# karenyang/GCN-VAE

Measured on AMD Instinct MI355X. Metric: edges/sec R-GCN forward+backward, FB15k-237 emb=200, higher is better.
Workload: dtype f32; 1 GPU; FB15k-237-shaped synthetic full graph (BASELINE configs[1]): 14541 entities, 474 directed relation types, E=544230 directed edges on this rank (544230 in the trained graph), 2-layer R-GCN-VAE bdd num_bases=100 emb_dim=200 dropout 0.2, 0 IAF blocks, DistMult decoder on T=220000 triplets per rank, step = fwd + loss(BCE+reg+KL+MMD) + bwd + clip + Adam; edges_per_gpu=544230, trained_graph_edges=544230, nodes=14541, triplets_per_gpu=220000, n_flows=0, gemm_precision=f32, launch=hipgraph, parallelism=single GPU, optimizer=replicated clip + Adam, k1_operands=f32

## Files before the change

gcn-vae_amd/lib.py:

```python
import ctypes
import os

import torch

_HERE = os.path.dirname(os.path.abspath(__file__))
LIB_PATH = os.path.join(_HERE, 'libgcnvae_hip.so')

_P, _I, _L, _F = ctypes.c_void_p, ctypes.c_int, ctypes.c_int64, ctypes.c_float

SIGNATURES = {
    'gv_version': (_I, []),
    'gv_last_error_string': (ctypes.c_char_p, []),
    'gv_index_caps': (None, [_L, _I, _I, _P, _P, _P]),
    'gv_index_workspace_bytes': (_L, [_L, _I]),
    'gv_build_csr': (_I, [_P, _L, _I, _I, _P, _P, _P, _I, _P, _I, _P, _L, _P]),
    'gv_build_csr_batch_workspace_bytes': (_L, [_P, _I]),
    'gv_build_csr_batch': (_I, [_P, _I, _P, _L, _P]),
    'gv_triplet_lists': (_I, [_P, _I, _L, _P, _P, _P, _P, _P, _P, _P, _P, _P]),
    'gv_widen2_i32': (_I, [_P, _P, _L, _P, _P, _L, _P]),
    'gv_graph_index_build': (_I, [_P, _P, _L, _I, _I, _I, _I, _P, _P, _P, _P, _I, _P, _I, _P, _P, _P, _P, _I, _P, _I, _P, _L, _P]),
    'gv_relation_index_build': (_I, [_P, _P, _P, _P, _P, _L, _I, _I, _P, _P, _P, _P, _P, _P, _P, _I, _P, _I, _P, _L, _P]),
    'gv_triplet_index_build': (_I, [_P, _L, _I, _I, _I, _I, _P, _P, _P, _P, _P, _I, _P, _I, _P, _P, _P, _P, _P, _I, _P, _I,
                                    _P, _L, _P]),
    'gv_perm_sample': (_I, [_L, _L, ctypes.c_uint64, ctypes.c_uint64, _P, _P, ctypes.c_uint32, _P, _P]),
    'gv_neighborhood_sample_workspace_bytes': (_L, [_I, _L]),
    'gv_neighborhood_sample': (_I, [_P, _P, _P, _P, _I, _L, _I, ctypes.c_uint64, ctypes.c_uint64, _P, ctypes.c_uint32, _P, _P, _L, _P]),
    'gv_relabel_workspace_bytes': (_L, [_I]),
    'gv_relabel_pairs': (_I, [_P, _P, _L, _I, _P, _I, _P, _P, _P, _P, _L, _P]),
    'gv_negative_sampling': (_I, [_P, _P, _P, _L, _I, _P, _P, _P, ctypes.c_uint64, ctypes.c_uint64, _P, ctypes.c_uint32, _P, _P, _P]),
    'gv_graph_from_triplets_workspace_bytes': (_L, [_L, _I, _I]),
    'gv_graph_from_triplets': (_I, [_P, _P, _P, _P, _L, _I, _I, _P, _P, _P, _P, _P, _L, _P]),
    'gv_segment_items_count': (_I, [_P, _I, _I, _P, _P, _P, _P]),
    'gv_segment_items_fill': (_I, [_P, _I, _I, _P, _P, _P, _P, _P, _P]),
    'gv_rgcn_bdd_aggregate': (_I, [_P, _I, _P, _I, _P, _P, _P, _P, _P, _I, _P, _I, _I, _I, _I, _I, _I,
                                   _P, _I, _I, _P, _F, _P, _I, _P, _P]),
    'gv_rgcn_bdd_phase_plan': (_I, [_I, _I, _I, _I, _I, _I, _I, _I, _I, _P]),
    'gv_rgcn_bdd_pack_weight_phase': (_I, [_P, _I, _I, _I, _I, _I, _P, _P]),
    'gv_rgcn_bdd_aggregate_phases': (_I, [_P, _P, _P, _P, _P, _I, _P, _I, _P, _I, _P, _I, _I, _I, _I, _I, _I, _I, _I, _I,
                                          _P, _I, _I, _P, _F, _P, _I, _P, _P]),
    'gv_rgcn_bdd_lds_plan': (_I, [_I, _I, _I, _I, _I, _P]),
    'gv_rgcn_bdd_pack_weight_lds': (_I, [_P, _I, _I, _I, _I, _I, _I, _P, _P]),
    'gv_rgcn_bdd_aggregate_lds': (_I, [_P, _I, _P, _P, _I, _P, _I, _P, _P, _P, _P, _P, _I, _P, _I, _I, _I, _I, _I, _P, _I, _I,
                                       _P, _F, _P, _I, _P, _I, _P]),
    'gv_rgcn_bdd_pack_supported': (_I, [_I, _I, _I, _I]),
    'gv_rgcn_bdd_pack_weight': (_I, [_P, _I, _I, _I, _I, _I, _P, _P]),
    'gv_rgcn_bdd_pack_weight_pair': (_I, [_P, _I, _I, _I, _I, _P, _P, _P]),
    'gv_rgcn_bdd_fixup': (_I, [_P, _I, _P, _I, _P, _I, _I, _P, _F, _P, _I, _P]),
    'gv_rgcn_bdd_grad_weight': (_I, [_P, _I, _P, _I, _P, _P, _P, _P, _P, _I, _P, _I, _I, _I, _I, _P, _P, _I, _P]),
    'gv_rgcn_epilogue_fwd': (_I, [_P, _P, _I, _P, _F, _P, _L, _I, _P]),
    'gv_rgcn_epilogue_bwd': (_I, [_P, _P, _I, _P, _F, _P, _L, _I, _P, _P]),
    'gv_colsum_finish': (_I, [_P, _I, _I, _P, _I, _P]),
    'gv_gemm_workspace_bytes': (_L, [_I, _I, _I, _I]),
    'gv_gemm_f32': (_I, [_I, _I, _I, _I, _I, _P, _I, _P, _I, _P, _I, _P, _I, _I, _I, _P, _P, _L, _P]),
    'gv_gemm_f32_live_rows': (_I, [_I, _I, _I, _I, _I, _P, _I, _P, _I, _P, _I, _P, _I, _I, _I, _P, _P, _L, _P, _P]),
    'gv_gemm_f32_sparse': (_I, [_I, _I, _I, _I, _I, _P, _I, _P, _I, _P, _I, _P, _I, _I, _I, _P, _P, _L, _P, _P, _P, _I, _P]),
    'gv_gemm_bf16': (_I, [_I, _I, _I, _I, _I, _P, _I, _P, _I, _P, _I, _P, _I, _I, _I, _P, _P, _L, _P]),
    'gv_gemm_bf16_nt_workspace_bytes': (_L, [_I, _I, _I]),
    'gv_gemm_bf16_gradw_fits': (_I, [_I, _I, _I, _I]),
    'gv_gemm_bf16_gradw_workspace_bytes': (_L, [_I, _I, _I]),
    'gv_gemm_bf16_gradw': (_I, [_P, _I, _P, _I, _I, _I, _I, _P, _I, _P, _I, _P, _L, _P]),
    'gv_gemm_bf16_gradw_tiles': (_I, [_P, _L, _P, _L, _I, _I, _I, _P, _I, _P, _I, _P, _L, _P]),
    'gv_gemm_bf16_nt': (_I, [_P, _I, _I, _P, _I, _I, _I, _I, _P, _I, _P, _I, _P, _I, _I, _P, _I, _P, _I, _I, _P, _L, _P]),
    'gv_cast_bf16': (_I, [_P, _I, _I, _I, _P, _I, _P, _I, _P]),
    'gv_rowsum_bf16_workspace_floats': (_L, [_I, _I]),
    'gv_iaf_update_fwd_bf16': (_I, [_P, _P, _I, _P, _P, _P, _P, _I, _P, _I, _L, _I, _P]),
    'gv_iaf_update_fwd_bf16_tiles': (_I, [_P, _P, _I, _P, _P, _P, _P, _I, _P, _L, _L, _I, _P]),
    'gv_iaf_update_bwd_bf16': (_I, [_P, _P, _I, _P, _P, _P, _P, _P, _I, _P, _I, _P, _L, _I, _P]),
    'gv_gather3_i32': (_I, [_P, _L, _P, _P, _P, _P, _P, _P, _P]),
    'gv_iaf_update_bwd_row0_workspace_floats': (_L, [_I]),
    'gv_iaf_update_bwd_row0': (_I, [_P, _P, _P, _P, _P, _P, _P, _P, _L, _I, _P]),
    'gv_iaf_update_bwd_bf16_ex': (_I, [_P, _P, _I, _P, _P, _P, _P, _P, _I, _P, _I, _P, _I, _L, _I, _P]),
    'gv_rowsum_bf16': (_I, [_P, _I, _I, _I, _P, _I, _P, _P]),
    'gv_rowsum_bf16_segments': (_I, [_P, _I, _I, _I, _I, _P, _P, _I, _P, _P]),
    'gv_made_pack_weight_elems': (_L, [_I, _I]),
    'gv_made_pack_weight': (_I, [_P, _I, _I, _I, _P, _P, _P]),
    'gv_made_pack_weight_multi': (_I, [_I, _P, _P, _P, _P, _P, _P, _P]),
    'gv_made_pack_weight_multi_iaf': (_I, [_I, _P, _P, _P, _P, _P, _P, _P]),
    'gv_made_pack_weight_iaf': (_I, [_P, _I, _I, _I, _P, _P]),
    'gv_made_chain_fits': (_I, [_I, _P, _P, _I]),
    'gv_made_chain': (_I, [_P, _I, _I, _I, _P, _P]),
    'gv_made_chain_iafb': (_I, [_P, _I, _I, _P, _P]),
    'gv_made_chain_fwd': (_I, [_P, _I, _I, _I, _P, _I, _P, _P]),
    'gv_made_chain_fwd_row0': (_I, [_P, _I, _I, _P, _I, _P, _P]),
    'gv_made_chain_debug_stamps': (_I, [_P]),
    'gv_made_pack_weight_f32_elems': (_L, [_I, _I]),
    'gv_made_pack_weight_f32_multi': (_I, [_I, _P, _P, _P, _P, _P, _P, _P]),
    'gv_made_chain_f32_fits': (_I, [_I, _P, _P]),
    'gv_made_chain_f32_plan': (_I, [_I, _P, _P, _P, _P, _P, _P, _P]),
    'gv_made_chain_f32': (_I, [_P, _I, _I, _I, _P, _P, _P, _P]),
    'gv_made_passes_f32': (_I, [_P, _I, _I, _I, _P, _P, _P, _P, _P]),
    'gv_made_gradw_f32_plan_words': (_L, [_I, _I]),
    'gv_made_gradw_f32_plan': (_I, [_P, _I, _I, _I, _P, _P]),
    'gv_made_gradw_f32_workspace_floats': (_L, [_I, _I, _L]),
    'gv_made_gradw_f32': (_I, [_P, _I, _P, _I, _I, _I, _L, _P, _P, _I, _P, _P, _P, _P, _I, _I, _P, _I, _P, _L, _P]),
    'gv_made_gradw_f32_multi_workspace_floats': (_L, [_I, _P]),
    'gv_made_gradw_f32_multi': (_I, [_I, _P, _P, _L, _P]),
    'gv_made_row_fwd': (_I, [_P, _I, _P, _P]),
    'gv_made_row_bwd': (_I, [_P, _I, _P, _P, _P]),
    'gv_rel_rows_gemm': (_I, [_P, _I, _P, _P, _I, _I, _I, _I, _P, _I, _P, _P]),
    'gv_rel_gradw_gemm': (_I, [_P, _I, _P, _P, _I, _P, _P, _P, _I, _I, _I, _P, _P]),
    'gv_rank_scores': (_I, [_P, _I, _P, _I, _P, _P, _P, _P, _I, _I, _I, _P]),
    'gv_rank_scores_filtered': (_I, [_P, _I, _P, _I, _P, _P, _P, _P, _P, _I, _P, _P, _P, _I, _I, _I, _P]),
    'gv_topk_scores_workspace_bytes': (_L, [_I, _I, _I]),
    'gv_topk_scores': (_I, [_P, _I, _P, _I, _P, _P, _P, _P, _I, _I, _P, _P, _P, _I, _I, _I, _P]),
    'gv_rank_scores_constrained': (_I, [_P, _I, _P, _I, _P, _P, _P, _P, _P, _I, _P, _I, _I, _P, _P, _P, _P, _P, _P, _I, _I, _I, _P]),
    'gv_topk_scores_constrained': (_I, [_P, _I, _P, _I, _P, _P, _P, _P, _I, _P, _I, _I, _P, _I, _P, _P, _P, _I, _I, _I, _P]),
    'gv_rank_scores_mc': (_I, [_P, _I, _L, _P, _I, _L, _I, _P, _P, _P, _P, _P, _I, _P, _P, _P, _I, _I, _I, _P]),
    'gv_topk_scores_mc': (_I, [_P, _I, _L, _P, _I, _L, _I, _P, _P, _P, _P, _I, _I, _P, _P, _P, _I, _I, _I, _P]),
    'gv_pair_prob_std_mc': (_I, [_P, _I, _L, _P, _I, _L, _I, _P, _P, _I, _P, _I, _I, _I, _P]),
    'gv_mine_scores_workspace_bytes': (_L, [_I, _I, _I]),
    'gv_mine_scores': (_I, [_P, _I, _P, _I, _P, _P, _P, _P, _I, _I, _I, ctypes.c_uint32, _I, ctypes.c_uint32, _I, _P, _L, _P, _P, _P, _L,
                            _I, _I, _I, _P]),
    'gv_mine_scores_typed': (_I, [_P, _I, _P, _I, _P, _P, _P, _P, _L, _P, _P, _P, _I, _I, _I, ctypes.c_uint32, _I, ctypes.c_uint32, _I,
                                  _P, _L, _P, _P, _I, _I, _I, _P]),
    'gv_mine_scores_typed_mc': (_I, [_P, _I, _L, _I, _P, _I, _P, _P, _P, _P, _L, _P, _P, _P, _I, _I, _I, ctypes.c_uint32, _I,
                                     ctypes.c_uint32, _I, _P, _L, _P, _P, _I, _I, _I, _P]),
    'gv_ec_basis_rows_fwd': (_I, [_P, _P, _P, _P, _L, _I, _I, _I, _L, _P, _P]),
    'gv_ec_basis_rows_bwd': (_I, [_P, _P, _P, _P, _P, _P, _L, _P, _P, _L, _I, _I, _I, _L, _P, _P, _P, _I, _P]),
    'gv_ec_head_fwd': (_I, [_P, _P, _P, _P, _L, _I, _P, _P, _P, _P, _P, _P]),
    'gv_ec_head_bwd': (_I, [_P, _P, _P, _P, _P, _P, _L, _I, _P, _P]),
    'gv_transe_sample': (_I, [_P, ctypes.c_uint32, _P, _L, _I, _P, _P, _P, _P, _P, _I, _I, _P, _P, _P, _P, _P]),
    'gv_transe_step': (_I, [_P, _P, _P, _P, _P, _I, _I, _I, _I, _I, _F, _F, _F, _P, _P, _P, _P, _P, _P]),
    'gv_transe_apply': (_I, [_P, _I, _P, _P, _P, _P, _I, _P, _P, _P, _I, _F, _P, _I, _F, _P, _P, _P]),
    'gv_transe_apply_opt': (_I, [_P, _I, _P, _P, _P, _P, _I, _P, _P, _P, _I, _I, ctypes.c_double, ctypes.c_double, ctypes.c_double,
                                 _P, _P, _P, _P, _P, _P, _I, _F, _P, _P, _P]),
    'gv_transe_queries': (_I, [_P, _P, _P, _P, _L, _I, _I, _I, _P, _P]),
    'gv_transe_distances': (_I, [_P, _L, _P, _I, _I, _I, _P, _P]),
    'gv_transe_rank_filtered': (_I, [_P, _L, _P, _I, _I, _I, _P, _P, _P, _P, _P, _P, _P]),
    'gv_transe_topk_workspace_bytes': (_L, [_L, _I, _I]),
    'gv_transe_topk': (_I, [_P, _L, _P, _I, _I, _I, _P, _P, _P, _I, _I, _P, _P, _P, _P]),
    'gv_transe_rank_constrained': (_I, [_P, _L, _P, _I, _I, _I, _P, _P, _P, _P, _P, _I, _I, _P, _P, _P, _P, _P, _P]),
    'gv_transe_topk_constrained': (_I, [_P, _L, _P, _I, _I, _I, _P, _P, _P, _I, _P, _I, _I, _P, _I, _P, _P, _P, _P]),
    'gv_transe_mine_workspace_bytes': (_L, [_I, _I, _I]),
    'gv_transe_mine': (_I, [_P, _P, _I, _I, _I, _I, _P, _P, _P, _I, _I, _I, ctypes.c_uint32, _I, ctypes.c_uint32, _I, _P, _L, _P, _P,
                            _P, _L, _P]),
    'gv_transe_mine_typed': (_I, [_P, _P, _I, _I, _I, _I, _P, _P, _P, _L, _P, _P, _P, _I, _I, _I, ctypes.c_uint32, _I, ctypes.c_uint32,
                                  _I, _P, _L, _P, _P, _P]),
    'gv_colsum': (_I, [_P, _P, _L, _I, _I, _P, _P, _I, _P]),
    'gv_gather_rows': (_I, [_P, _P, _P, _L, _I, _P]),
# ... 102 lines not shown
```

gcn-vae_amd/ops.py:

```python
import contextlib
import ctypes as _ct
import itertools as _it
import os as _os
from dataclasses import dataclass
from typing import Optional

import torch

from . import lib
from .lib import ptr

ACT_NONE, ACT_RELU = 0, 1

DIRECT_GRAD = {}
GRAD_FRESH = set()
DIRECT_EPOCH = [0]


def _stamp_direct(ctx):
    ctx._gv_direct_epoch = DIRECT_EPOCH[0]


def _verify_direct(ctx):
    if getattr(ctx, '_gv_direct_epoch', DIRECT_EPOCH[0]) != DIRECT_EPOCH[0]:
# ... 891 lines not shown

MINE_TYPED_SPAN = 8
MINE_TYPED_FILL = 1024


def mine_typed_plan(ptr, num_rels, span=None, multiple=1):
    sizes = (ptr[1:] - ptr[:-1]).to(torch.int64)
    n_o, n_s = sizes[:num_rels], sizes[num_rels:]
    s_tiles, o_tiles = (n_s + 63) // 64, (n_o + 63) // 64
    if span is None:
        pairs = int((s_tiles * o_tiles).sum())
        span = min(MINE_TYPED_SPAN, max(1, pairs // MINE_TYPED_FILL))
        span = max(multiple, span // multiple * multiple)
    span = int(span)
    if span < 1:
        raise ValueError(f'span must be >= 1, got {span}')
    groups = (o_tiles + span - 1) // span
    per_r = s_tiles * groups
    total = int(per_r.sum())
    if total > 2 ** 31 - 1:
        raise ValueError(f'the type-constrained sweep has {total} units, more than 2**31 - 1')
    rel = torch.repeat_interleave(torch.arange(num_rels, device=ptr.device), per_r)
    local = torch.arange(total, device=ptr.device) - (torch.cumsum(per_r, 0) - per_r)[rel]
    g = groups[rel].clamp(min=1)
    first = (local % g) * span
    units = torch.stack([rel, local // g, first, torch.minimum(first + span, o_tiles[rel])], 1)
    return units.to(torch.int32).contiguous()


def _mine_typed_members(ptr, ids, n, num_rels):
    for name, t in (('ptr', ptr), ('ids', ids)):
        if not isinstance(t, torch.Tensor) or t.dim() != 1 or t.dtype not in (torch.int32, torch.int64):
            raise TypeError(f'{name}: expected a 1-D int32 / int64 tensor')
    if ptr.numel() != 2 * num_rels + 1:
        raise ValueError(f'ptr: expected {2 * num_rels + 1} entries (2 R + 1), got {ptr.numel()}')
    if ids.device != ptr.device:
        raise ValueError('ptr and ids must be on one device')
    ptr = ptr.to(torch.int64)
    if int(ptr[0]) != 0 or bool((ptr[1:] < ptr[:-1]).any()) or int(ptr[-1]) != ids.numel():
        raise ValueError(f'ptr must start at 0, be non-decreasing and end at ids.numel() = {ids.numel()}')
    if ids.numel() >= 2 ** 31:
        raise ValueError('ids: more than 2**31 - 1 members')
    if ids.numel():
        if int(ids.min()) < 0 or int(ids.max()) >= n:
            raise ValueError(f'member ids must lie in [0, {n})')
        starts = torch.zeros(ids.numel() + 1, dtype=torch.bool, device=ids.device)
        starts[ptr] = True
        if bool(((ids[1:] <= ids[:-1]) & ~starts[1:-1]).any()):
            raise ValueError('the members of every set must be strictly ascending')
    return ptr.contiguous(), ids.to(torch.int32).contiguous()


def _mine_typed_filter_args(filt_lo, filt_hi, filt_ent, n, num_rels, dev):
    lo32, hi32, ent32, n_ent, _, _ = _mine_filter_args(filt_lo, filt_hi, filt_ent, n, num_rels, dev, lambda *a: 0)
    if n_ent > 1:
        starts = torch.zeros(n_ent + 1, dtype=torch.bool, device=dev)
        starts[lo32.long()] = True
        if bool(((ent32[1:] < ent32[:-1]) & ~starts[1:-1]).any()):
            raise ValueError('the listed objects of every key must be ascending')
    return lo32, hi32, ent32, n_ent


def mine_scores_typed(emb, w, set_ptr, set_ids, *, threshold=None, k=None, bias=None, filt_lo=None, filt_hi=None, filt_ent=None,
                      exclude_self=True, max_results=MINE_MAX_RESULTS, span=None):
    return _mine_scores('gv_mine_scores_typed', emb, w, (set_ptr, set_ids, span), threshold, k, bias, filt_lo, filt_hi, filt_ent,
                        exclude_self, max_results)


def mine_scores_typed_mc(z, w, set_ptr, set_ids, *, threshold=None, k=None, bias=None, filt_lo=None, filt_hi=None, filt_ent=None,
                         exclude_self=True, max_results=MINE_MAX_RESULTS, span=None):
    return _mine_scores('gv_mine_scores_typed_mc', z, w, (set_ptr, set_ids, span), threshold, k, bias, filt_lo, filt_hi, filt_ent,
                        exclude_self, max_results, mc=True)


def pick_split_k(m_out, n_out, k):
    tiles = ((m_out + 63) // 64) * ((n_out + 63) // 64)
    if tiles >= 256 or k < 2048:
        return 1
    if k >= 65536:
        return 64
    return max(1, min(64, 1024 // tiles, k // 256))


def colsum(x, out=None, accumulate=False, relu_mask=None):
    x, ld = _row_major(x, 'x')
    if relu_mask is not None:
        relu_mask, ldm = _row_major(relu_mask, 'relu_mask')
        if tuple(relu_mask.shape) != tuple(x.shape) or ldm != ld:
            raise ValueError('relu_mask must have the shape and leading dimension of x')
    m, n = x.shape
    if out is None:
        out = torch.empty(n, dtype=torch.float32, device=x.device)
        accumulate = False
    ws = torch.empty(64 * n, dtype=torch.float32, device=x.device)
    lib.call('gv_colsum', ptr(x), ptr(relu_mask), m, n, ld, ptr(out), ptr(ws), 1 if accumulate else 0, lib.stream())
    return out


def epilogue_fwd(agg, addend, act, keep, keep_scale):
    agg = _chk(agg, name='agg')
    out = torch.empty_like(agg)
    if addend is not None:
        addend = _chk(addend, name='addend')
    lib.call('gv_rgcn_epilogue_fwd', ptr(agg), ptr(addend), act, ptr(keep), float(keep_scale), ptr(out),
             agg.shape[0], agg.shape[1], lib.stream())
    return out


def epilogue_bwd(out, grad_out, act, keep, keep_scale, colsum_out=None, colsum_accumulate=False):
    grad_out = _chk(grad_out.contiguous(), name='grad_out')
    g = torch.empty_like(grad_out)
    m, n = grad_out.shape
    fused = colsum_out is not None and n % 4 == 0 and n <= 1024
    part = torch.empty(EPILOGUE_COLSUM_SLICES * n, dtype=torch.float32, device=g.device) if fused else None
    lib.call('gv_rgcn_epilogue_bwd', ptr(out), ptr(grad_out), act, ptr(keep), float(keep_scale), ptr(g), m, n, ptr(part),
             lib.stream())
    if fused:
        lib.call('gv_colsum_finish', ptr(part), n, EPILOGUE_COLSUM_SLICES, ptr(colsum_out), 1 if colsum_accumulate else 0,
                 lib.stream())
    elif colsum_out is not None:
        colsum(g, out=colsum_out, accumulate=colsum_accumulate)
    return g


def axpby(alpha, x, beta=0.0, y=None, a=None):
    x = _chk(x.contiguous(), name='x')
    if y is None:
        y = torch.empty_like(x)
        beta = 0.0
    lib.call('gv_axpby', x.numel(), ptr(a), float(alpha), ptr(x), float(beta), ptr(y), lib.stream())
    return y


def copy_into(dst, src):
    src = _chk(src.contiguous(), name='src')
    if dst.numel() != src.numel() or not dst.is_contiguous():
        raise ValueError('copy_into: same size, contiguous destination')
    lib.call('gv_axpby', src.numel(), None, 1.0, ptr(src), 0.0, ptr(dst), lib.stream())
    return dst


def copy_of(x):
    return copy_into(torch.empty_like(x, memory_format=torch.contiguous_format), x)


class _CatRows(torch.autograd.Function):

    @staticmethod
    def forward(ctx, a, b):
        out = torch.empty(a.shape[0] + b.shape[0], a.shape[1], dtype=torch.float32, device=a.device)
        copy_into(out[:a.shape[0]], a)
        copy_into(out[a.shape[0]:], b)
        ctx.na = a.shape[0]
        return out

    @staticmethod
    def backward(ctx, g):
        return g[:ctx.na], g[ctx.na:]


def cat_rows(a, b):
    return _CatRows.apply(a, b)


class _SplitRows(torch.autograd.Function):

# ... 140 lines not shown

class _EmbeddingIdentity(torch.autograd.Function):

    @staticmethod
    def forward(ctx, table, tick_rng):
        ctx.set_materialize_grads(False)
        if tick_rng is not None:
            tick_rng.tick()
        ctx.direct = _direct(table)
        _stamp_direct(ctx)
        return table.detach().view(table.shape)

    @staticmethod
    def backward(ctx, g):
        if g is None:
            return None, None
        g = _chk(g.contiguous(), name='grad')
        _verify_direct(ctx)
        tgt = ctx.direct
        if tgt is None:
            return g, None
        lib.call('gv_axpby', g.numel(), None, 1.0, ptr(g), 1.0, ptr(tgt), lib.stream())
        GRAD_FRESH.discard(tgt.data_ptr())
        return None, None


_identity_ids = {}


def _ids_are_identity(table, ids):
    if ids.numel() != table.shape[0]:
        return False
    key = (ids.data_ptr(), ids._version, ids.numel())
    hit = _identity_ids.get(key)
    if hit is None:
        if len(_identity_ids) > 64:
            _identity_ids.clear()
        hit = _identity_ids[key] = (bool((ids.reshape(-1) == torch.arange(ids.numel(), device=ids.device)).all()), ids)
    return hit[0]


def embedding(table, ids, tick_rng=None, sole_consumer=False):
    identity = False
    if table.is_cuda and isinstance(ids, torch.Tensor) and ids.is_cuda and ids.dtype == torch.int64:
        if torch.cuda.is_current_stream_capturing():
            hit = _identity_ids.get((ids.data_ptr(), ids._version, ids.numel()))
            identity = bool(hit and hit[0]) and ids.numel() == table.shape[0]
        else:
            identity = _ids_are_identity(table, ids)
    if identity and sole_consumer:
        out = _EmbeddingIdentity.apply(table, tick_rng)
        out._gv_grad_target = _direct(table)
        return out
    return _Embedding.apply(table, ids, tick_rng)


def _epilogue_grad(out, grad_out, act, keep, keep_scale, want_bias, d_b):
    if not want_bias:
        return epilogue_bwd(out, grad_out, act, keep, keep_scale), None
    grad_bias = d_b if d_b is not None else torch.empty(grad_out.shape[1], dtype=torch.float32, device=grad_out.device)
    g = epilogue_bwd(out, grad_out, act, keep, keep_scale, colsum_out=grad_bias, colsum_accumulate=d_b is not None)
    return g, (None if d_b is not None else grad_bias)


def _gemm_addend(x, loop_weight, h_bias, out_feat, loop_bf=None):
    if loop_weight is not None and loop_bf is not None:
        return dense_bf16(x, loop_bf[0], loop_weight.shape[1], loop_weight.shape[0], bias=h_bias)
    if loop_weight is not None:
        return gemm(x, loop_weight, bias=h_bias)
    if h_bias is not None:
        return h_bias.unsqueeze(0).expand(x.shape[0], out_feat).contiguous()
    return None


def _row_addend(h_bias, loop_rows, n, out_feat):
    if h_bias is None:
        return loop_rows
    addend = h_bias.unsqueeze(0).expand(n, out_feat).contiguous()
    if loop_rows is not None:
        lib.call('gv_axpby', addend.numel(), None, 1.0, ptr(loop_rows), 1.0, ptr(addend), lib.stream())
    return addend


def _loop_grads(x, g, loop_weight, d_l, want_loop, want_x, loop_bf=None):
    if loop_weight is None:
        return None, None
    grad_loop = gx_loop = None
    if want_loop:
        grad_loop = gemm(x, g, trans_a=True, split_k=pick_split_k(x.shape[1], g.shape[1], x.shape[0]), out=d_l,
                         accumulate=d_l is not None)
        if d_l is not None:
            grad_loop = None
    if want_x:
        if loop_bf is not None:
            gx_loop = dense_bf16(g, loop_bf[1], loop_weight.shape[0], loop_weight.shape[1])
        else:
            gx_loop = gemm(g, loop_weight, trans_b=True)
    return grad_loop, gx_loop


def _coef_order(gidx, ridx, coef, side):
    if gidx.sync_free or coef is None:
        return coef, (gidx.by_src.perm if side == 'src' else ridx.by_rel.perm)
    return (gidx.coef_in_src_order(coef) if side == 'src' else ridx.coef_in_rel_order(coef)), None


def _relation_weight_grad(gidx, ridx, coef, x, g, nb, si, so, d_w):
    coef_r, idx_r = _coef_order(gidx, ridx, coef, 'rel')
    grad_w = bdd_grad_weight(ridx.by_rel.seg, ridx.src_by_rel, ridx.dst_by_rel, coef_r, idx_r, x, g, nb, si, so, out=d_w,
                             accumulate=d_w is not None)
    return None if d_w is not None else grad_w


def _bdd_weight_fwd(ctx, weight, nb, si, so, pk, pk_bwd):
    ctx.w_bwd_packed = None
    ctx.w_version = weight._version
    if pk and pk_bwd:
        w_fwd, ctx.w_bwd_packed = torch.empty_like(weight), torch.empty_like(weight)
        lib.call('gv_rgcn_bdd_pack_weight_pair', ptr(weight), weight.shape[0], nb, si, so, ptr(w_fwd), ptr(ctx.w_bwd_packed),
                 lib.stream())
        return w_fwd
    return pack_weight(weight, nb, si, so, False) if pk else weight


def _bdd_weight_bwd(ctx, weight, nb, so, si):
    pk = si * so >= 8 and pack_supported(nb, so, si, True)
    if ctx.w_bwd_packed is not None and weight._version == ctx.w_version:
        return ctx.w_bwd_packed, pk
    return (pack_weight(weight, nb, so, si, True) if pk else weight), pk


def _bdd_k1(ctx, side, tl, gidx, ridx, coef, feat, weight, nb, bi, bo, plain_weight, addend, act=ACT_NONE, keep=None,
            keep_scale=1.0, out=None, sharded=False):
    trans, r = side == 'src', weight.shape[0]
    if tl is not None:
        return bdd_aggregate_phases(tl, None if coef is None else tl.coef(coef), feat, pack_weight_phase(tl, weight, nb, bi, bo),
                                    r, nb, bi, bo, addend(), act, keep, keep_scale, out=out)
    seg = gidx.by_src.seg if trans else gidx.by_dst.seg
    nbr, ety = (gidx.nbr_by_src, ridx.et_by_src) if trans else (gidx.nbr_by_dst, ridx.et_by_dst)

    def coef_operands():
        return _coef_order(gidx, ridx, coef, 'src') if trans else (coef, gidx.by_dst.perm)
    lp = None if (ctx.grouped or sharded) else lds_plan(r, nb, bi, bo, bf=ctx.k1_bf if trans else None)
    if lp is not None and lds_graph(gidx, side, lp[2]):
        if not trans:
            ctx.k1_bf = bool(lp[3])
            if not torch.cuda.is_current_stream_capturing():
                lp_b = lds_plan(r, nb, bo, bi, bf=ctx.k1_bf)
                if lp_b is not None:
                    gidx.lds_order('src', lp_b[2])
        c, c_idx = coef_operands()
        return bdd_aggregate_lds(gidx.lds_order(side, lp[2]), nbr, ety, c, c_idx, feat,
                                 pack_weight_lds(weight, nb, bi, bo, trans, lp), r, nb, bi, bo, trans, addend(), act, keep,
                                 keep_scale, out=out, plan=lp)
    w, pk = plain_weight()
    if ctx.grouped:
        seg_g, nbr_g, ety_g, perm = ridx.grouped_order(gidx, side)
        coef_g = None if coef is None else ridx.grouped_coef(coef, side, perm)
        return bdd_aggregate(seg_g, nbr_g, ety_g, coef_g, None, feat, w, nb, bi, bo, trans, addend(), act, keep, keep_scale,
                             out=out, packed=pk)
    if K1_REL_RUNS and not gidx.sync_free and not sharded:
        nbr_r, et_r, _, coef_r = ridx.rel_sorted(gidx, side, coef)
        return bdd_aggregate(_k1_items(gidx, seg), nbr_r, et_r, coef_r, None, feat, w, nb, bi, bo, trans, addend(), act, keep,
                             keep_scale, out=out, packed=pk)
    c, c_idx = coef_operands()
    return bdd_aggregate(_k1_items(gidx, seg), nbr, ety, c, c_idx, feat, w, nb, bi, bo, trans, addend(), act, keep, keep_scale,
                         out=out, packed=pk)


class _RelGraphConvBdd(torch.autograd.Function):

    @staticmethod
    def forward(ctx, x, weight, h_bias, loop_weight, norm, gidx, ridx, num_bases, act, keep, keep_scale,
# ... 1710 lines not shown
```

include/gcnvae.h:

```cpp
#ifndef GCNVAE_H
#define GCNVAE_H

#include <stdint.h>

#ifdef __cplusplus
extern "C" {
#endif

typedef enum {
    GV_OK = 0,
    GV_ERR_NULL = -1,
    GV_ERR_SHAPE = -2,
    GV_ERR_ALIGN = -3,
    GV_ERR_WORKSPACE = -4
} gv_status;

enum { GV_ACT_NONE = 0, GV_ACT_RELU = 1 };

int gv_version(void);
const char* gv_last_error_string(void);

int gv_segment_items_count(const int32_t* rowptr, int n_seg, int chunk, int32_t* n_chunks, int32_t* n_slots,
                           int32_t* is_split, void* stream);
int gv_segment_items_fill(const int32_t* rowptr, int n_seg, int chunk, const int32_t* item_off,
// ... 252 lines not shown

int gv_mine_scores_typed_mc(const float* e, int ld_e, int64_t e_stride, int n_samples, const float* w, int ld_w, const float* bias,
                            const int64_t* set_ptr, const int32_t* set_ids, const int32_t* units, int64_t n_units,
                            const int32_t* filt_lo, const int32_t* filt_hi, const int32_t* filt_ent, int n_filt_ent,
                            int exclude_self, int mode, uint32_t key_min, int prefix_bits, uint32_t prefix, int bin_bits,
                            int32_t* out, int64_t capacity, uint64_t* counter, uint64_t* hist, int n, int num_rels, int h,
                            void* stream);

#define GV_EC_HEAD_MAX_CLASSES 64
int gv_ec_basis_rows_fwd(const float* v, const float* comp, const int32_t* run_id, const int32_t* run_rel, int64_t n_runs, int h,
                         int nb, int num_rels, int64_t rows, float* msg, void* stream);
int gv_ec_basis_rows_bwd(const float* v, const float* comp, const float* s, const int32_t* run_id, const int32_t* run_rel,
                         const int64_t* run_ptr, int64_t n_groups, const int64_t* q_pos, const int64_t* rel_ptr, int64_t n_runs,
                         int h, int nb, int num_rels, int64_t rows, float* dv, float* q, float* dcomp, int accumulate, void* stream);
int gv_ec_head_fwd(const float* h, const int64_t* labels, const int32_t* row_pos, const int64_t* set_off, int64_t n, int c,
                   float* p, float* term, int32_t* correct, float* loss, int32_t* count, void* stream);
int gv_ec_head_bwd(const float* p, const int64_t* labels, const int32_t* row_pos, const int64_t* set_off, const float* gloss,
                   const float* grad_p, int64_t n, int c, float* dh, void* stream);

#define GV_TRANSE_MAX_DIM 512
int gv_transe_sample(const uint64_t* rng_state, uint32_t stream_id, const int32_t* train, int64_t n_train, int n_ent,
                     const float* p_head, const int32_t* f_lo, const int32_t* f_hi, const int32_t* f_ent_o, const int32_t* f_ent_s,
                     int batch, int neg_ent, int32_t* bh, int32_t* br, int32_t* bt, uint32_t* draws, void* stream);
int gv_transe_step(const float* ent, const float* rel, const int32_t* bh, const int32_t* br, const int32_t* bt, int batch, int neg_ent,
                   int dim, int p_norm, int norm_flag, float margin, float adv_temperature, float regul_rate, float* g_ent,
                   float* g_rel, float* loss_part, float* score, int32_t* occ_ent, void* stream);
int gv_transe_apply(float* ent, int n_ent, const float* g_ent, const int32_t* perm_e, const int32_t* rowptr_e, float* rel, int n_rel,
                    const float* g_rel, const int32_t* perm_r, const int32_t* rowptr_r, int dim, float lr, const float* loss_part,
                    int batch, float margin, float* loss_out, double* epoch_acc, void* stream);
#define GV_TRANSE_OPT_SGD 0
#define GV_TRANSE_OPT_ADAGRAD 1
#define GV_TRANSE_OPT_ADADELTA 2
#define GV_TRANSE_OPT_ADAM 3
int gv_transe_apply_opt(float* ent, int n_ent, const float* g_ent, const int32_t* perm_e, const int32_t* rowptr_e, float* rel,
                        int n_rel, const float* g_rel, const int32_t* perm_r, const int32_t* rowptr_r, int dim, int method, double lr,
                        double weight_decay, double lr_decay, float* s1_ent, float* s2_ent, float* s1_rel, float* s2_rel,
                        const int64_t* step_t, const float* loss_part, int batch, float margin, float* loss_out, double* epoch_acc,
                        void* stream);
int gv_transe_queries(const float* ent, const float* rel, const int32_t* a, const int32_t* r, int64_t m, int dim, int head,
                      int norm_flag, float* q, void* stream);
int gv_transe_distances(const float* q, int64_t m, const float* en, int v, int dim, int p_norm, float* out, void* stream);
int gv_transe_rank_filtered(const float* q, int64_t m, const float* en, int v, int dim, int p_norm, const int32_t* target,
                            const int32_t* f_lo, const int32_t* f_hi, const int32_t* f_ent, int32_t* counts_raw, int32_t* counts_filt,
                            void* stream);
int64_t gv_transe_topk_workspace_bytes(int64_t m, int v, int k);
int gv_transe_topk(const float* q, int64_t m, const float* en, int v, int dim, int p_norm, const int32_t* filt_lo,
                   const int32_t* filt_hi, const int32_t* filt_ent, int n_filt_ent, int k, int64_t* out_ids, float* out_dist,
                   void* workspace, void* stream);
int gv_transe_rank_constrained(const float* q, int64_t m, const float* en, int v, int dim, int p_norm, const int32_t* target,
                               const int32_t* f_lo, const int32_t* f_hi, const int32_t* f_ent, const uint32_t* cand, int ld_cand,
                               int n_sets, const int32_t* cand_set, int32_t* counts_raw, int32_t* counts_filt, int32_t* counts_raw_c,
                               int32_t* counts_filt_c, void* stream);
int gv_transe_topk_constrained(const float* q, int64_t m, const float* en, int v, int dim, int p_norm, const int32_t* filt_lo,
                               const int32_t* filt_hi, const int32_t* filt_ent, int n_filt_ent, const uint32_t* cand, int ld_cand,
                               int n_sets, const int32_t* cand_set, int k, int64_t* out_ids, float* out_dist, void* workspace,
                               void* stream);

int64_t gv_transe_mine_workspace_bytes(int n, int num_rels, int n_filt_ent);
int gv_transe_mine(const float* en, const float* rn, int n, int num_rels, int dim, int p_norm, const int32_t* filt_lo,
                   const int32_t* filt_hi, const int32_t* filt_ent, int n_filt_ent, int exclude_self, int mode, uint32_t key_min,
                   int prefix_bits, uint32_t prefix, int bin_bits, int32_t* out, int64_t capacity, uint64_t* counter, uint64_t* hist,
                   void* workspace, int64_t workspace_bytes, void* stream);

int gv_transe_mine_typed(const float* en, const float* rn, int n, int num_rels, int dim, int p_norm, const int64_t* set_ptr,
                         const int32_t* set_ids, const int32_t* units, int64_t n_units, const int32_t* filt_lo,
                         const int32_t* filt_hi, const int32_t* filt_ent, int n_filt_ent, int exclude_self, int mode,
                         uint32_t key_min, int prefix_bits, uint32_t prefix, int bin_bits, int32_t* out, int64_t capacity,
                         uint64_t* counter, uint64_t* hist, void* stream);

int64_t gv_gemm_workspace_bytes(int m, int n, int k, int split_k);
int gv_gemm_f32(int trans_a, int trans_b, int m, int n, int k, const float* a, int lda, const float* b, int ldb,
                float* c, int ldc, const float* bias, int act, int accumulate, int split_k, const float* a_relu_mask,
                void* workspace, int64_t workspace_bytes, void* stream);
int gv_gemm_f32_live_rows(int trans_a, int trans_b, int m, int n, int k, const float* a, int lda, const float* b, int ldb, float* c,
                          int ldc, const float* bias, int act, int accumulate, int split_k, const float* a_relu_mask, void* workspace,
                          int64_t workspace_bytes, const int32_t* rows_dev, void* stream);
int gv_gemm_f32_sparse(int trans_a, int trans_b, int m, int n, int k, const float* a, int lda, const float* b, int ldb, float* c,
                       int ldc, const float* bias, int act, int accumulate, int split_k, const float* a_relu_mask, void* workspace,
                       int64_t workspace_bytes, const int32_t* rows_dev , const uint64_t* b_k_chunks,
                       const uint64_t* c_tiles, int c_tiles_wanted, void* stream);
int gv_gemm_bf16(int trans_a, int trans_b, int m, int n, int k, const float* a, int lda, const float* b, int ldb,
                float* c, int ldc, const float* bias, int act, int accumulate, int split_k, const float* a_relu_mask,
                void* workspace, int64_t workspace_bytes, void* stream);

int gv_colsum(const float* x, const float* relu_mask, int64_t m, int n, int ld, float* out, float* workspace,
              int accumulate, void* stream);

int gv_gather_rows(const float* table, const int64_t* ids, float* out, int64_t n, int h, void* stream);
int gv_gather_rows_rng_tick(const float* table, const int64_t* ids, float* out, int64_t n, int h, uint64_t* rng_state,
                            void* stream);
int gv_scatter_add_rows(const float* grad_out, const int64_t* ids, float* grad_table, int64_t n, int h, void* stream);

#define GV_RNG_MAX_JOBS 8
#define GV_RNG_KEEP_MASK 0
#define GV_RNG_NORMAL 1
int gv_rng_fill(const uint64_t* rng_state, int n_jobs, void* const* ptrs, const int64_t* counts, const int32_t* kinds,
                const float* drop_p, const uint32_t* streams, void* stream);
int gv_rng_tick(uint64_t* rng_state, void* stream);

int gv_reparam_fwd(const float* h2, const float* eps, float* z, float* v, float* m_out ,
                   int64_t n, int h, void* stream);
int gv_reparam_bwd(const float* h2, const float* eps, const float* v, const float* gz, const float* gm,
                   const float* gv, float* grad_h2, int64_t n, int h, void* stream);

int gv_distmult_bce_fwd(const float* embed, int ld_e, const float* w_rel, int ld_w, const int32_t* triplets,
                        const int32_t* order ,
                        const float* labels, const float* bias, float* score, float* loss, float* workspace,
                        int64_t t, int h, void* stream);
int gv_bce_grad(const float* score, const float* labels, const float* gloss, float* dscore,
                const int32_t* pos3 , float* dscore_inc , float* dscore_rel ,
                float* dbias, float* workspace, int64_t t, void* stream);

int gv_distmult_bce_fwd_grad(const int32_t* items, int n_items, const int32_t* rel_s, const int32_t* rel_o,
                             const int32_t* rel_tid, const float* embed, int ld_e, const float* w_rel, int ld_w,
                             const float* labels, const float* bias, const int32_t* pos3, float* score, float* delta,
                             float* u, float* partial, float* workspace, int64_t t, int h, void* stream);
int gv_distmult_grad_finish(const float* gloss, const float* u, const float* partial, const int32_t* fix, int n_fix,
                            const int32_t* rowptr, int chunk, int num_rels, int h, const float* w_rel, int ld_w,
                            float reg_scale, float* grad_w, int ld_gw, int accumulate, const float* delta, float* d_out,
                            int64_t n_coef, const float* workspace, float* dbias, int64_t t, void* stream);

int gv_mean_sq(const float* x, int64_t n, float scale, float* out, float* workspace, int accumulate, void* stream);
int gv_mean_sq2(const float* x1, int64_t n1, float scale1, const float* x2, int64_t n2, float scale2, float* out,
                float* workspace, const int32_t* rows_dev, int64_t rows_host, void* stream);
int gv_axpby(int64_t n, const float* a, float alpha, const float* x, float beta, float* y, void* stream);
int gv_mul(int64_t n, const float* a, const float* b, float* out, void* stream);
#define GV_MUL_MULTI_MAX 8
int gv_mul_multi(int count, const float* const* a, const float* const* b, float* const* out, const int64_t* n, void* stream);
int64_t gv_kl_workspace_bytes(int64_t n, int h, int k);
int gv_kl_fwd(const float* z, const float* m, int ld_m, const float* v, const float* z_pre, const float* flp,
              float* resp, float* kl, float* workspace, int64_t n, int h, int k, const int32_t* rows_dev, void* stream);
int gv_kl_bwd(const float* z, const float* m, int ld_m, const float* v, const float* z_pre, const float* resp,
              const float* gkl, float gscale, float z_extra, float* gz, float* gm, float* gv, float* g_zpre,
              int accumulate_zpre, float* workspace, int mix_ready, int64_t n, int h, int k, const int32_t* rows_dev,
              void* stream);
int gv_reparam_kl_fwd(const float* h2, const float* eps, const float* z_pre, float* z, float* v, float* m_out, float* resp,
                      float* workspace, int64_t n, int h, int k, void* stream);
int gv_reparam_kl_bwd(const float* z, const float* h2, const float* v, const float* eps, const float* z_pre, const float* resp,
                      const float* gkl, float gscale, float z_extra, const float* gz_up, float* gh2, float* g_zpre,
                      int accumulate_zpre, float* workspace, int64_t n, int h, int k, void* stream);

int gv_loss_combine(const float* ws_pred, int64_t t, const float* ws_reg, int64_t n_embed, int64_t n_wrel,
                    const float* ws_kl, int64_t n_nodes, int h, int k, const float* ws_mmd, int sx, int sy, float reg_w,
                    float kl_w, float mmd_w, float* scal , float* loss, const int32_t* rows_dev,
                    void* stream);
int gv_lincomb4(const float* a0, float c0, const float* a1, float c1, const float* a2, float c2, const float* a3,
                float c3, float* out, void* stream);
int gv_mmd_fwd(const float* x, const float* y, const int64_t* y_index, int sx, int sy, int h, float* mmd, float* workspace,
               void* stream);
int gv_mmd_bwd(const float* x, const float* y, const int64_t* y_index, int sx, int sy, int h, const float* gmmd, float gscale,
               float* gx, float* gy, void* stream);
int gv_prior_sample_fwd(const float* z_pre, const float* eps, float* out, int s, int k, int h, void* stream);
int gv_prior_sample_bwd(const float* z_pre, const float* eps, const float* g, float* gz_pre, int accumulate, int s, int k,
                        int h, void* stream);

int gv_iaf_update_fwd(const float* z, const float* net, int ld_net, const float* x_old, const int32_t* colcount,
                      float* x_new, int64_t n, int d, void* stream);
int gv_iaf_update_bwd(const float* z, const float* net, int ld_net, const int32_t* colcount, const float* g_xnew,
                      const float* g_logdet , float* g_z, float* g_net, float* g_xold, int64_t n, int d,
                      void* stream);
int gv_iaf_update_bwd_acc(const float* z, const float* net, int ld_net, const int32_t* colcount, const float* g_xnew,
                          const float* g_logdet, float* g_z, int gz_accumulate, float* g_net, float* g_xold, int64_t n, int d,
                          void* stream);
int gv_rowsum(const float* x, int ld, int col0, int ncols, float* out, int64_t n, void* stream);
int gv_reverse_cols(const float* x, float* out, int64_t n, int d, void* stream);
int gv_mean_rows_multi(int count, const float* const* x, int64_t n, const int32_t* rows_dev, float* out, float* workspace,
// ... 74 lines not shown
```

Before: 576.9 million edges/s.

## Add split-K MFMA tall-skinny TN GEMM for self-loop weight gradients

Adds a dedicated f32 kernel for A^T·B with a small output dimension (m ≤ 224) and a very long K (the node count). Each block owns a 32-column output strip, and eight waves split K, each accumulating with 32x32x2 f32 MFMA into register accumulators. The waves' partials are reduced through LDS, with an optional cross-block split-K pass that sums into a workspace. It replaces the generic split-K GEMM for the self-loop weight gradient when no relu mask is used, aiming at better CU utilisation on this tall-skinny shape, at the cost of extra workspace traffic and an additional sum kernel.

Measured after the change: 583.1 million edges/s, median of 6. No clear change (+1.1%).

```diff
diff --git a/gcn-vae_amd/csrc/k_gemm_tall.hip b/gcn-vae_amd/csrc/k_gemm_tall.hip
--- /dev/null
+++ b/gcn-vae_amd/csrc/k_gemm_tall.hip
@@ -0,0 +1,233 @@
+#include <stdlib.h>
+
+#include <algorithm>
+
+#include "common.h"
+
+namespace gv {
+
+typedef float f32x16 __attribute__((ext_vector_type(16)));
+
+constexpr int TT_WAVES = 8;
+constexpr int TT_D = 4;
+constexpr int TT_MAX_MT = 7;
+constexpr int TT_MAX_SPLIT = 64;
+
+struct TallParams {
+    const float* a;
+    const float* b;
+    float* c;
+    float* ws;
+    int m, n, k, lda, ldb, ldc;
+    int split, accumulate;
+    const int* rows_dev;
+};
+
+__device__ __forceinline__ int tall_live_k(const TallParams& p) {
+    int kl = p.k;
+    if (p.rows_dev) kl = max(0, min(kl, *p.rows_dev));
+    return kl;
+}
+
+template <int MT>
+__global__ __launch_bounds__(64 * TT_WAVES) void k_gemm_tn_tall(const TallParams p) {
+    __shared__ float red[TT_WAVES][2][1024];
+    const int lane = threadIdx.x & 63, wid = __builtin_amdgcn_readfirstlane(threadIdx.x >> 6);
+    const int l31 = lane & 31, lhi = lane >> 5;
+    const int kl = tall_live_k(p);
+    if (kl == 0 && p.accumulate) return;
+
+    const int ncol = (p.n + 31) >> 5;
+    int v = blockIdx.x;
+    {
+        const int total = gridDim.x, q = total >> 3, r = total & 7, xcd = v & 7, j = v >> 3;
+        v = (xcd < r ? xcd * (q + 1) : r * (q + 1) + (xcd - r) * q) + j;
+    }
+    const int z = v / ncol, ct = v - z * ncol;
+
+    const int steps = (kl + 1) >> 1;
+    const int nsub = p.split * TT_WAVES;
+    const int per = (steps + nsub - 1) / nsub;
+    const int sub = z * TT_WAVES + wid;
+    const int kb = (int)min((long long)kl, 2ll * sub * per), ke = (int)min((long long)kl, kb + 2ll * per);
+    const int nfull = (ke - kb) >> 1;
+    const bool odd = (ke - kb) & 1;
+
+    f32x16 acc[MT];
+#pragma unroll
+    for (int t = 0; t < MT; ++t)
+#pragma unroll
+        for (int i = 0; i < 16; ++i) acc[t][i] = 0.f;
+
+    if (ke > kb) {
+        int aoff[MT];
+#pragma unroll
+        for (int t = 0; t < MT; ++t) aoff[t] = min(32 * t + l31, p.m - 1);
+        const int boff = min(32 * ct + l31, p.n - 1);
+        auto load_step = [&](int s, float (&xa)[MT], float& xb) {
+            const int row = min(kb + 2 * s + lhi, ke - 1);
+            const float* ar = p.a + (size_t)row * p.lda;
+            const float* br = p.b + (size_t)row * p.ldb;
+#pragma unroll
+            for (int t = 0; t < MT; ++t) xa[t] = ar[aoff[t]];
+            xb = br[boff];
+        };
+        float ra[TT_D][MT], rb[TT_D], ta[MT], tb;
+#pragma unroll
+        for (int d = 0; d < TT_D; ++d) load_step(d, ra[d], rb[d]);
+        load_step(nfull, ta, tb);
+        int cur = max(0, min(TT_D, nfull - 1));
+        const float* pa = p.a + (size_t)(kb + 2 * cur + lhi) * p.lda + l31;
+        const float* pl = p.a + (size_t)(kb + 2 * cur + lhi) * p.lda + aoff[MT - 1];
+        const float* pb = p.b + (size_t)(kb + 2 * cur + lhi) * p.ldb + boff;
+        int it = 0;
+        for (; it + TT_D <= nfull; it += TT_D) {
+#pragma unroll
+            for (int d = 0; d < TT_D; ++d) {
+#pragma unroll
+                for (int t = 0; t < MT; ++t) {
+                    acc[t] = __builtin_amdgcn_mfma_f32_32x32x2f32(ra[d][t], rb[d], acc[t], 0, 0, 0);
+                    if (t + 1 < MT) {
+                        ra[d][t] = pa[32 * t];
+                    } else {
+                        ra[d][t] = *pl;
+                        rb[d] = *pb;
+                    }
+                    __builtin_amdgcn_sched_barrier(0);
+                }
+                const bool more = cur + 1 < nfull;
+                const size_t sa = more ? 2 * (size_t)p.lda : 0, sb = more ? 2 * (size_t)p.ldb : 0;
+                pa += sa; pl += sa; pb += sb;
+                cur += more;
+            }
+        }
+        const int rest = nfull - it;
+#pragma unroll
+        for (int d = 0; d < TT_D - 1; ++d)
+            if (d < rest) {
+#pragma unroll
+                for (int t = 0; t < MT; ++t) acc[t] = __builtin_amdgcn_mfma_f32_32x32x2f32(ra[d][t], rb[d], acc[t], 0, 0, 0);
+            }
+        if (odd) {
+            const float bz = lhi ? 0.f : tb;
+#pragma unroll
+            for (int t = 0; t < MT; ++t) acc[t] = __builtin_amdgcn_mfma_f32_32x32x2f32(lhi ? 0.f : ta[t], bz, acc[t], 0, 0, 0);
+        }
+    }
+
+#pragma unroll
+    for (int t0 = 0; t0 < MT; t0 += 2) {
+        if (t0) __syncthreads();
+#pragma unroll
+        for (int u = 0; u < 2; ++u)
+            if (t0 + u < MT) {
+#pragma unroll
+                for (int i = 0; i < 16; ++i) red[wid][u][i * 64 + lane] = acc[t0 + u][i];
+            }
+        __syncthreads();
+        constexpr int PER_THREAD = 2 * 1024 / (64 * TT_WAVES);
+#pragma unroll
+        for (int e = 0; e < PER_THREAD; ++e) {
+            const int idx = e * 64 * TT_WAVES + threadIdx.x;
+            const int u = idx >> 10, reg = (idx >> 6) & 15, ln = idx & 63;
+            if (t0 + u >= MT) continue;
+            const float* src = &red[0][0][0] + idx;
+            const float s = ((src[0] + src[2048]) + (src[2 * 2048] + src[3 * 2048])) +
+                            ((src[4 * 2048] + src[5 * 2048]) + (src[6 * 2048] + src[7 * 2048]));
+            const int row = 32 * (t0 + u) + (reg & 3) + 8 * (reg >> 2) + 4 * (ln >> 5), col = 32 * ct + (ln & 31);
+            if (row >= p.m || col >= p.n) continue;
+            if (p.split > 1) {
+                p.ws[((size_t)z * p.m + row) * p.n + col] = s;
+            } else {
+                float* dst = p.c + (size_t)row * p.ldc + col;
+                *dst = p.accumulate ? *dst + s : s;
+            }
+        }
+    }
+}
+
+__global__ __launch_bounds__(256) void k_gemm_tn_tall_sum(const TallParams p) {
+    if (p.accumulate && tall_live_k(p) == 0) return;
+    const int total = p.m * p.n;
+    const int i = blockIdx.x * 256 + threadIdx.x;
+    if (i >= total) return;
+    const int row = i / p.n, col = i - row * p.n;
+    float* dst = p.c + (size_t)row * p.ldc + col;
+    const float old = p.accumulate ? *dst : 0.f;
+    float a0 = 0.f, a1 = 0.f, a2 = 0.f, a3 = 0.f;
+    for (int z0 = 0; z0 < p.split; z0 += 16) {
+        float t[16];
+#pragma unroll
+        for (int q = 0; q < 16; ++q) t[q] = p.ws[(size_t)min(z0 + q, p.split - 1) * total + i];
+#pragma unroll
+        for (int q = 0; q < 16; q += 4) {
+            a0 += z0 + q < p.split ? t[q] : 0.f;
+            a1 += z0 + q + 1 < p.split ? t[q + 1] : 0.f;
+            a2 += z0 + q + 2 < p.split ? t[q + 2] : 0.f;
+            a3 += z0 + q + 3 < p.split ? t[q + 3] : 0.f;
+        }
+    }
+    const float s = (a0 + a1) + (a2 + a3);
+    *dst = p.accumulate ? old + s : s;
+}
+
+}
+
+using namespace gv;
+
+extern "C" int gv_gemm_f32_tn_tall_fits(int m, int n, int k) {
+    return m >= 1 && m <= 32 * TT_MAX_MT && n >= 1 && k >= 0 && (long long)m * n <= INT32_MAX / 2;
+}
+
+extern "C" int gv_gemm_f32_tn_tall_split(int m, int n, int k) {
+    (void)m;
+    static const int env = getenv("GV_GEMM_TALL_SPLIT") ? atoi(getenv("GV_GEMM_TALL_SPLIT")) : 0;
+    if (env > 0) return std::min(env, TT_MAX_SPLIT);
+    if (n < 1 || k < 1) return 1;
+    const int ncol = (n + 31) / 32;
+    const int by_cus = current_device_cus() / ncol, by_k = k / (2 * 8 * TT_WAVES);
+    return std::max(1, std::min(TT_MAX_SPLIT, std::min(by_cus, by_k)));
+}
+
+extern "C" int64_t gv_gemm_f32_tn_tall_workspace_bytes(int m, int n, int split) {
+    return split > 1 ? (int64_t)split * m * n * (int64_t)sizeof(float) : 0;
+}
+
+extern "C" int gv_gemm_f32_tn_tall(int m, int n, int k, const float* a, int lda, const float* b, int ldb, float* c, int ldc,
+                                   int accumulate, int split, void* workspace, int64_t workspace_bytes, const int32_t* rows_dev,
+                                   void* stream) {
+    GV_REQUIRE(m >= 0 && n >= 0 && k >= 0, GV_ERR_SHAPE, "gv_gemm_f32_tn_tall: negative size");
+    if (m == 0 || n == 0) return GV_OK;
+    GV_REQUIRE(gv_gemm_f32_tn_tall_fits(m, n, k), GV_ERR_SHAPE, "gv_gemm_f32_tn_tall: m=%d n=%d beyond the kernel (m <= %d)", m, n,
+               32 * TT_MAX_MT);
+    GV_REQUIRE(c && (k == 0 || (a && b)), GV_ERR_NULL, "gv_gemm_f32_tn_tall: NULL matrix");
+    GV_REQUIRE(lda >= m && ldb >= n && ldc >= n, GV_ERR_SHAPE, "gv_gemm_f32_tn_tall: leading dimension too small (lda=%d ldb=%d ldc=%d)",
+               lda, ldb, ldc);
+    GV_REQUIRE(split >= 1 && split <= TT_MAX_SPLIT, GV_ERR_SHAPE, "gv_gemm_f32_tn_tall: split=%d outside [1, %d]", split, TT_MAX_SPLIT);
+    if (split > 1) {
+        GV_REQUIRE(workspace, GV_ERR_NULL, "gv_gemm_f32_tn_tall: split > 1 needs a workspace");
+        GV_REQUIRE(workspace_bytes >= gv_gemm_f32_tn_tall_workspace_bytes(m, n, split), GV_ERR_WORKSPACE,
+                   "gv_gemm_f32_tn_tall: workspace %lld < %lld bytes", (long long)workspace_bytes,
+                   (long long)gv_gemm_f32_tn_tall_workspace_bytes(m, n, split));
+    }
+    TallParams p;
+    p.a = a; p.b = b; p.c = c; p.ws = (float*)workspace;
+    p.m = m; p.n = n; p.k = k; p.lda = lda; p.ldb = ldb; p.ldc = ldc;
+    p.split = split; p.accumulate = accumulate ? 1 : 0;
+    p.rows_dev = rows_dev;
+    hipStream_t st = (hipStream_t)stream;
+    const dim3 grid(((n + 31) / 32) * split), block(64 * TT_WAVES);
+    switch ((m + 31) / 32) {
+        case 1: hipLaunchKernelGGL(k_gemm_tn_tall<1>, grid, block, 0, st, p); break;
+        case 2: hipLaunchKernelGGL(k_gemm_tn_tall<2>, grid, block, 0, st, p); break;
+        case 3: hipLaunchKernelGGL(k_gemm_tn_tall<3>, grid, block, 0, st, p); break;
+        case 4: hipLaunchKernelGGL(k_gemm_tn_tall<4>, grid, block, 0, st, p); break;
+        case 5: hipLaunchKernelGGL(k_gemm_tn_tall<5>, grid, block, 0, st, p); break;
+        case 6: hipLaunchKernelGGL(k_gemm_tn_tall<6>, grid, block, 0, st, p); break;
+        default: hipLaunchKernelGGL(k_gemm_tn_tall<7>, grid, block, 0, st, p); break;
+    }
+    int rc = launch_status("gv_gemm_f32_tn_tall");
+    if (rc != GV_OK || split == 1) return rc;
+    hipLaunchKernelGGL(k_gemm_tn_tall_sum, dim3((m * n + 255) / 256), dim3(256), 0, st, p);
+    return launch_status("gv_gemm_f32_tn_tall(sum)");
+}
diff --git a/gcn-vae_amd/lib.py b/gcn-vae_amd/lib.py
--- a/gcn-vae_amd/lib.py
+++ b/gcn-vae_amd/lib.py
@@ -55,6 +55,10 @@
     'gv_gemm_f32_live_rows': (_I, [_I, _I, _I, _I, _I, _P, _I, _P, _I, _P, _I, _P, _I, _I, _I, _P, _P, _L, _P, _P]),
     'gv_gemm_f32_sparse': (_I, [_I, _I, _I, _I, _I, _P, _I, _P, _I, _P, _I, _P, _I, _I, _I, _P, _P, _L, _P, _P, _P, _I, _P]),
     'gv_gemm_bf16': (_I, [_I, _I, _I, _I, _I, _P, _I, _P, _I, _P, _I, _P, _I, _I, _I, _P, _P, _L, _P]),
+    'gv_gemm_f32_tn_tall_fits': (_I, [_I, _I, _I]),
+    'gv_gemm_f32_tn_tall_split': (_I, [_I, _I, _I]),
+    'gv_gemm_f32_tn_tall_workspace_bytes': (_L, [_I, _I, _I]),
+    'gv_gemm_f32_tn_tall': (_I, [_I, _I, _I, _P, _I, _P, _I, _P, _I, _I, _I, _P, _L, _P, _P]),
     'gv_gemm_bf16_nt_workspace_bytes': (_L, [_I, _I, _I]),
     'gv_gemm_bf16_gradw_fits': (_I, [_I, _I, _I, _I]),
     'gv_gemm_bf16_gradw_workspace_bytes': (_L, [_I, _I, _I]),
diff --git a/gcn-vae_amd/ops.py b/gcn-vae_amd/ops.py
--- a/gcn-vae_amd/ops.py
+++ b/gcn-vae_amd/ops.py
@@ -997,6 +997,45 @@
     return max(1, min(64, 1024 // tiles, k // 256))
 
 
+LOOP_GRADW_TALL = _os.environ.get('GV_LOOP_GRADW_TALL', '1') == '1'
+GEMM_TALL_MAX_M = 224
+
+
+def gemm_tn_tall(a, b, out=None, accumulate=False, split=None):
+    a, lda = _row_major(a, 'a')
+    b, ldb = _row_major(b, 'b')
+    (k, m), (kb, n) = a.shape, b.shape
+    if k != kb:
+        raise ValueError(f'gemm_tn_tall inner dimensions differ: {k} vs {kb}')
+    if b.device != a.device:
+        raise ValueError(f'b must be on the device of a ({a.device}), got {b.device}')
+    if m * n and not lib.load().gv_gemm_f32_tn_tall_fits(m, n, k):
+        raise ValueError(f'gemm_tn_tall: m={m} beyond the kernel (m <= {GEMM_TALL_MAX_M})')
+    if out is None:
+        out = torch.empty(m, n, dtype=torch.float32, device=a.device)
+        accumulate = False
+    else:
+        if not isinstance(out, torch.Tensor) or out.dtype != torch.float32 or out.dim() != 2:
+            raise TypeError(f'out: expected a 2-D float32 tensor, got {getattr(out, "dtype", type(out).__name__)} '
+                            f'{tuple(getattr(out, "shape", ()))}')
+        if out.device != a.device:
+            raise ValueError(f'out must be on the device of a ({a.device}), got {out.device}')
+        if tuple(out.shape) != (m, n):
+            raise ValueError(f'out: expected shape {(m, n)}, got {tuple(out.shape)}')
+        if m * n and ((n > 1 and out.stride(1) != 1) or (m > 1 and out.stride(0) < n)):
+            raise ValueError(f'out: needs unit inner stride and a leading dimension >= {n}, got strides {out.stride()}')
+    if m * n == 0:
+        return out
+    split = int(lib.load().gv_gemm_f32_tn_tall_split(m, n, k)) if split is None else int(split)
+    ws_bytes = int(lib.load().gv_gemm_f32_tn_tall_workspace_bytes(m, n, split))
+    ws = torch.empty(ws_bytes // 4, dtype=torch.float32, device=a.device) if ws_bytes else None
+    live = LIVE_ROWS
+    rows = live[0] if (live is not None and k == live[1] and a.device == live[0].device) else None
+    lib.call('gv_gemm_f32_tn_tall', m, n, k, ptr(a), lda, ptr(b), ldb, ptr(out), out.stride(0) if m > 1 else n,
+             1 if accumulate else 0, split, ptr(ws), ws_bytes, ptr(rows), lib.stream(), tag=f'loopgradwtall_{m}x{n}_nb1')
+    return out
+
+
 def colsum(x, out=None, accumulate=False, relu_mask=None):
     x, ld = _row_major(x, 'x')
     if relu_mask is not None:
@@ -1303,13 +1342,17 @@
     return addend
 
 
-def _loop_grads(x, g, loop_weight, d_l, want_loop, want_x, loop_bf=None):
+def _loop_grads(x, g, loop_weight, d_l, want_loop, want_x, loop_bf=None, x_relu_mask=None):
     if loop_weight is None:
         return None, None
     grad_loop = gx_loop = None
     if want_loop:
-        grad_loop = gemm(x, g, trans_a=True, split_k=pick_split_k(x.shape[1], g.shape[1], x.shape[0]), out=d_l,
-                         accumulate=d_l is not None)
+        if (LOOP_GRADW_TALL and GEMM_PRECISION == 'f32' and x_relu_mask is None and x.dim() == 2 and g.dim() == 2
+                and 1 <= x.shape[1] <= GEMM_TALL_MAX_M and g.shape[1] >= 1):
+            grad_loop = gemm_tn_tall(x, g, out=d_l, accumulate=d_l is not None)
+        else:
+            grad_loop = gemm(x, g, trans_a=True, split_k=pick_split_k(x.shape[1], g.shape[1], x.shape[0]), out=d_l,
+                             accumulate=d_l is not None, a_relu_mask=x_relu_mask)
         if d_l is not None:
             grad_loop = None
     if want_x:
diff --git a/include/gcnvae.h b/include/gcnvae.h
--- a/include/gcnvae.h
+++ b/include/gcnvae.h
@@ -358,6 +358,11 @@
 int gv_gemm_bf16(int trans_a, int trans_b, int m, int n, int k, const float* a, int lda, const float* b, int ldb,
                 float* c, int ldc, const float* bias, int act, int accumulate, int split_k, const float* a_relu_mask,
                 void* workspace, int64_t workspace_bytes, void* stream);
+int gv_gemm_f32_tn_tall_fits(int m, int n, int k);
+int gv_gemm_f32_tn_tall_split(int m, int n, int k);
+int64_t gv_gemm_f32_tn_tall_workspace_bytes(int m, int n, int split);
+int gv_gemm_f32_tn_tall(int m, int n, int k, const float* a, int lda, const float* b, int ldb, float* c, int ldc, int accumulate,
+                        int split, void* workspace, int64_t workspace_bytes, const int32_t* rows_dev , void* stream);
 
 int gv_colsum(const float* x, const float* relu_mask, int64_t m, int n, int ld, float* out, float* workspace,
               int accumulate, void* stream);
```
